# rvolden/C3POa

Measured on AMD Instinct MI355X. Metric: R2C2 reads->consensus/sec, higher is better.
Workload: dtype int32

## Files before the change

c3poa_amd/csrc/c3_args.h:

```cpp
#pragma once
#include "c3_dev.h"
#include <cstddef>

struct C3Counters {
  int queue;
  int peaks_queue;
  unsigned long long cells;
  unsigned long long cells_computed;
  unsigned long long zero_cells;
  int poa_ovf;
  int poa_ovf16;
  int n_windows;
  int win_ovf;
  int win_queue2;
  int band_layers, band_fallback;
  int band_mismatch;
  struct { int window, layer, R, q, band_row, full_row, next_row; } verify;
  unsigned long long phases[16];
};
static_assert(offsetof(C3Counters, cells) % 8 == 0 && offsetof(C3Counters, cells_computed) % 8 == 0 &&
              offsetof(C3Counters, zero_cells) % 8 == 0 && offsetof(C3Counters, phases) % 8 == 0, "u64 counters must be 8-byte aligned");

struct ConkArgs {
  C3Batch b; const uint8_t* sp_codes; const int* sp_len; int32_t* track; C3Info* info; C3Counters* cnt;
// ... 17 lines not shown
  int* overflow;
  int* overflow16;
};
#define C3_POA_NI 19
__host__ __device__ inline int c3_poa_far_shift(bool w32) { return w32 ? 0 : 2; }
struct PoaLayout { size_t ints, edges, cells, bases, score, desc, jump, path, total; };
__host__ __device__ inline PoaLayout c3_poa_layout(size_t Ncap, size_t K, int cells_cap, int far_shift, size_t Pcap) {
  PoaLayout l;
  l.ints = sizeof(int) * C3_POA_NI * Ncap; l.edges = sizeof(int) * 3 * Ncap * K;
  l.cells = 2 * (size_t)cells_cap + 16 * (size_t)(cells_cap >> far_shift);
  l.bases = 5 * Ncap; l.score = sizeof(long long) * Ncap; l.desc = sizeof(uint4) * 2 * Ncap;
  l.jump = sizeof(int) * C3_JUMP_LEVELS * Ncap; l.path = sizeof(int) * Pcap;
  l.total = l.ints + l.edges + l.cells + l.bases + l.score + l.desc + l.jump + l.path;
  return l;
}

struct WLayer { int qbeg, len, begin, end; };
struct WinRec { int rid, w, n_layers, blen, tgs, out_len, polished, pad_; };
struct PrepArgs {
  C3Batch b; C3Info* info; C3Params p; C3Counters* cnt; const int* work; int n_work;
  const uint8_t* draft; int32_t* tpos; int wcap; uint8_t* eD; int64_t ecap; int* lw_first; int* lw_last; int NLcap, NWcap;
  WinRec* wrec; WLayer* wlay; int* win_base;
  int sub_shift;
  int rows_old;
};
struct WinArgs {
  C3Batch b; C3Params p; C3Counters* cnt; int n_win; const WinRec* wrec_in; WinRec* wrec; const WLayer* wlay; int NLcap;
  const uint8_t* draft;
  uint8_t* base; int* ibase; int* ebase; long long* score;
  int32_t* H; uint16_t* D; uint4* rdesc; int Ncap, K; long long hcap; uint8_t* wout; int wout_cap;
  int Lcap;
  int band_mode;
  const int* wlist; int* ovf_list;
};
#define W_INTS 19
struct WinLayout { size_t ints, edges, bases, score, H, D, desc, total; };
__host__ __device__ inline WinLayout c3_win_layout(size_t Ncap, size_t K, size_t hcap) {
  WinLayout l;
  l.ints = sizeof(int) * W_INTS * Ncap; l.edges = sizeof(int) * 4 * Ncap * K; l.bases = 2 * Ncap; l.score = sizeof(long long) * Ncap;
  l.H = sizeof(int32_t) * hcap; l.D = hcap; l.desc = sizeof(uint4) * (Ncap + 1);
  l.total = l.ints + l.edges + l.bases + l.score + l.H + l.D + l.desc;
  return l;
}
struct StitchArgs {
  C3Batch b; C3Info* info; const int* work; int n_work; const WinRec* wrec; const int* win_base; const uint8_t* wout; int wout_cap; char* cons;
  const uint8_t* zflag;
};
struct AdapterArgs {
  C3Batch b; C3Params p; C3Counters* cnt;
  const uint8_t* ad_codes; const int* ad_len; int n_ad;
  uint8_t* D; long long dcap;
  int32_t* out;
};

struct ZeroArgs {
  C3Batch b; C3Info* info; C3Params p; C3Counters* cnt; const int* work; int n_work;
  uint8_t* D; long long dcap;
  int4* zinfo; uint8_t* zflag;
  const uint8_t* draft; char* cons;
  uint8_t* S; long long scap; int zk;
};

struct ZlLayout { long long ck, dir, car, total; };
__host__ __device__ inline ZlLayout c3_zl_layout(long long n0, long long n1, long long K) {
  ZlLayout l;
  l.ck = 0;
// ... 15 lines not shown
```

c3poa_amd/csrc/c3_stages.hip:

```cpp
#include "c3_host.h"

__global__ void k_summary(const C3Info* info, const int64_t* off, int n, Summary* out) {
  int i = blockIdx.x * blockDim.x + threadIdx.x;
  if (i >= n) return;
  const C3Info* p = &info[i];
  Summary s; s.status = p->status; s.n_sub = p->n_sub; s.max_sub = 0; s.sum_sub = 0; s.max_dang = 0; s.n_peaks = p->n_peaks;
  for (int k = 0; k < p->n_sub; ++k) { int l = p->sub_end[k] - p->sub_beg[k]; s.sum_sub += l; if (l > s.max_sub) s.max_sub = l; }
  int L = (int)(off[i + 1] - off[i]);
  s.front = p->has_front ? p->front_end : 0; s.tail = p->has_tail ? L - p->tail_beg : 0;
  if (p->has_front) s.max_dang = p->front_end;
  if (p->has_tail && L - p->tail_beg > s.max_dang) s.max_dang = L - p->tail_beg;
  out[i] = s;
}

static hipError_t zero_counters(c3_handle* h) { return hipMemsetAsync(h->d_counter.p, 0, sizeof(C3Counters), h->stream); }

static int auto_slots(c3_handle* h, int want, size_t per_slot_bytes, int n_items, int waves_per_cu) {
  int s = want > 0 ? want : h->n_cus * waves_per_cu;
  size_t budget = h->mem_total ? h->mem_total / 3 : ((size_t)64 << 30);
  if (per_slot_bytes > 0) { size_t mx = budget / per_slot_bytes; if ((size_t)s > mx) s = (int)std::max<size_t>(mx, 1); }
  if (s > n_items) s = std::max(n_items, 1);
  return s;
}

// ... 285 lines not shown
  h->n_windows = n_win;
  DBG("prep done: n_win=%d\n", n_win);
  const int wout_cap = 3 * WL + 64;
  HIPCHK(hipEventRecord(h->ev[7], h->stream));
  if (n_win > 0) {
    HIPCHK(h->d_wout.ensure((size_t)n_win * wout_cap));
    const int Ncap = 3 * WL + 40 * NLcap, K = NLcap + 2;
    const long long hcap_full = (long long)(Ncap + 1) * 64 * 12;
    const int R_typ = std::min(Ncap, WL + WL / 4 + 30 * NLcap + 64);
    long long hcap = std::min(hcap_full, (long long)(R_typ + R_typ / 2 + 4) * 256);
    if (const char* e = getenv("C3_DEBUG_HCAP_DIV")) hcap = std::max(4096LL, hcap_full / std::max(1, atoi(e)) / 64 * 64);
    const WinLayout L = c3_win_layout(Ncap, K, hcap), L2 = c3_win_layout(Ncap, K, hcap_full);
    const int slots = auto_slots(h, h->cfg.slots_win, L.total, n_win, 20);
    const int slots2 = hcap < hcap_full ? std::min(slots, 256) : 0;
    const size_t S = (size_t)slots, S2 = (size_t)slots2;
    HIPCHK(h->s_win_i.ensure(L.ints * S + 64)); HIPCHK(h->s_win_nk.ensure(L.edges * S));
    HIPCHK(h->s_win_h.ensure(L.H * S)); HIPCHK(h->s_win_d.ensure(L.D * S + 256));
    HIPCHK(h->s_win_b.ensure(L.bases * S)); HIPCHK(h->s_win_sc.ensure(L.score * S)); HIPCHK(h->s_win_desc.ensure(L.desc * S));
    if (slots2) {
      HIPCHK(h->s_win_h2.ensure(L2.H * S2)); HIPCHK(h->s_win_d2.ensure(L2.D * S2 + 256));
      HIPCHK(h->d_wovf.ensure(sizeof(int) * (size_t)n_win));
    }
    WinArgs a; memset(&a, 0, sizeof(a));
    a.b = dev_batch(h); a.p = dev_params(h->cfg); a.cnt = dev_cnt(h); a.n_win = n_win;
    a.wrec_in = h->d_wrec.as<WinRec>(); a.wrec = h->d_wrec.as<WinRec>(); a.wlay = h->d_wlay.as<WLayer>(); a.NLcap = NLcap;
    a.draft = h->d_draft.as<uint8_t>();
    a.ibase = h->s_win_i.as<int>(); a.ebase = h->s_win_nk.as<int>();
    a.base = h->s_win_b.as<uint8_t>(); a.score = h->s_win_sc.as<long long>();
    a.H = h->s_win_h.as<int32_t>(); a.D = h->s_win_d.as<uint16_t>(); a.rdesc = h->s_win_desc.as<uint4>(); a.Ncap = Ncap; a.K = K; a.hcap = hcap; a.Lcap = std::min(std::min(Ncap, 2 * WL + 30 * NLcap), ((getenv("C3_DEBUG_WIN_LDS") ? atoi(getenv("C3_DEBUG_WIN_LDS")) : 6656) - 16) / 6);
    if (const char* e = getenv("C3_DEBUG_WIN_LCAP")) a.Lcap = std::max(64, std::min(Ncap, atoi(e)));
    a.wout = h->d_wout.as<uint8_t>(); a.wout_cap = wout_cap;
    HIPCHK(zero_counters(h));
    if (const char* e = getenv("C3_DEBUG_BAND")) a.band_mode = !strcmp(e, "off") ? 1 : !strcmp(e, "fail") ? 2 : !strcmp(e, "verify") ? 3 : 0;
    a.ovf_list = slots2 ? h->d_wovf.as<int>() : nullptr;
    c3k_launch_window(&a, slots, h->stream);
    HIPCHK(hipGetLastError());
    if (slots2) {
      a.H = h->s_win_h2.as<int32_t>(); a.D = h->s_win_d2.as<uint16_t>(); a.hcap = hcap_full;
      a.wlist = h->d_wovf.as<int>(); a.ovf_list = nullptr;
      c3k_launch_window(&a, slots2, h->stream);
      HIPCHK(hipGetLastError());
    }
    HIPCHK(hipMemcpyAsync(h->phase_win, dev_cnt(h)->phases, sizeof(h->phase_win), hipMemcpyDeviceToHost, h->stream));
  }
  HIPCHK(hipEventRecord(h->ev[8], h->stream));
  StitchArgs s; memset(&s, 0, sizeof(s));
  s.b = dev_batch(h); s.info = h->d_info.as<C3Info>(); s.work = h->d_work.as<int>(); s.n_work = nw;
  s.wrec = h->d_wrec.as<WinRec>(); s.win_base = h->d_wbase.as<int>(); s.wout = h->d_wout.as<uint8_t>(); s.wout_cap = wout_cap;
  s.cons = h->d_cons.as<char>(); s.zflag = h->d_zflag.as<uint8_t>();
  DBG("stitch\n");
  c3k_launch_stitch(&s, std::min(nw, h->n_cus * 16), h->stream);
  HIPCHK(hipGetLastError());
  HIPCHK(hipEventRecord(h->ev[9], h->stream));
  HIPCHK(read_counters(h, &c));
  if (n_win > 0) {
    h->tm.n_win_redo = c.win_ovf; h->tm.cells_polish += c.cells; h->tm.cells_polish_computed += c.cells_computed;
    h->tm.n_band_layers = c.band_layers; h->tm.n_band_fallback = c.band_fallback; h->tm.n_band_mismatch = c.band_mismatch;
    if (c.band_mismatch) fprintf(stderr, "c3poa: band verify mismatch in window %d layer %d (R = %d): last differing base q = %d, band row %d, full row %d, row of q+1 = %d\n",
                                 c.verify.window, c.verify.layer, c.verify.R, c.verify.q, c.verify.band_row, c.verify.full_row, c.verify.next_row);
  }
  HIPCHK(hipEventElapsedTime(ms_prep, h->ev[5], h->ev[6]));
  HIPCHK(hipEventElapsedTime(ms_win, h->ev[7], h->ev[8]));
  HIPCHK(hipEventElapsedTime(ms_st, h->ev[8], h->ev[9]));
  h->tm.n_windows = n_win;
  return 0;
}
// ... 102 lines not shown
```

c3poa_amd/csrc/k_polish.hip:

```cpp
#include "c3_dev.h"
#include "c3_args.h"
#include "c3_launch.h"
#include <algorithm>
#include <type_traits>

#define WSYNC() __syncthreads()
#define EI(v, k) ((size_t)(k) * (size_t)c.Ncap + (size_t)(v))
#ifndef C3_WIN_RING
#define C3_WIN_RING 1
#endif



#ifndef C3_PREP_WAVES
#define C3_PREP_WAVES 5
#endif
#define EC 5
#define EXT_DCAP 4096
#define EXT_STATIC (-(1 << 27))
#define EXT_ECW 8
__device__ inline long long ext_dir_bytes(long long n, int rpw) { return (n / rpw + 1) * 256; }
template <bool DL>
__device__ long long extend_align(const PrepArgs& a, const uint32_t* pk, const uint8_t* draft, const uint8_t* ldraft, int C,
                                  int pb, int n, int dir_, int32_t* tpos, uint8_t* D, int lane) {
// ... 349 lines not shown
  __device__ __forceinline__ WArr<int> order2() const { return {I, (unsigned)(4 - osel) * (unsigned)Ncap}; }
  __device__ __forceinline__ WArr<int> lob() const { return {I, 17u * (unsigned)Ncap + 8u}; }
#undef W_I
  __device__ __forceinline__ WArr<int> in_from() const { return {E, 0u}; }
  __device__ __forceinline__ WArr<int> in_w() const { return {E, (unsigned)Ncap * (unsigned)K}; }
  __device__ __forceinline__ WArr<int> out_to() const { return {E, 2u * (unsigned)Ncap * (unsigned)K}; }
  __device__ __forceinline__ WArr<int> out_w() const { return {E, 3u * (unsigned)Ncap * (unsigned)K}; }
  __device__ __forceinline__ WArr<uint8_t> base() const { return {B8, 0u}; }
  __device__ __forceinline__ WArr<uint8_t> mask() const { return {B8, (unsigned)Ncap}; }
};

#ifndef WU
#define WU 4
#endif
__device__ void w_blocks(WCtx& c, int lane) {
  int gprev = -1;
  for (int i0 = 0; i0 < c.n; i0 += 64 * WU) {
    int v[WU], r[WU];
#pragma unroll
    for (int u = 0; u < WU; ++u) { const int i = i0 + 64 * u + lane; v[u] = i < c.n ? c.order()[i] : -1; }
#pragma unroll
    for (int u = 0; u < WU; ++u) r[u] = v[u] >= 0 ? c.grp()[v[u]] : -2;
#pragma unroll
    for (int u = 0; u < WU; ++u) {
      const int i = i0 + 64 * u + lane;
      const int rp = wave_shr1(r[u], gprev);
      gprev = wave_bcast(r[u], 63);
      if (v[u] >= 0 && r[u] != rp) { c.gfirst()[r[u]] = i; if (i > 0) c.glast()[rp] = i - 1; }
      if (v[u] >= 0 && i + 1 == c.n) c.glast()[r[u]] = i;
    }
  }
  WSYNC();
}
__device__ void w_reorder(WCtx& c, int n_old, int lane, int* lds, int lds_cap) {
  const int n_new = c.n - n_old;
  const bool inl = n_new <= lds_cap;
  if (inl) { for (int k = lane; k < n_new; k += 64) lds[k] = c.anchor()[k]; WSYNC(); }
  for (int i0 = 0; i0 < n_old; i0 += 64 * WU) {
    int v[WU];
#pragma unroll
    for (int u = 0; u < WU; ++u) { const int i = i0 + 64 * u + lane; v[u] = i < n_old ? c.order()[i] : -1; }
#pragma unroll
    for (int u = 0; u < WU; ++u) {
      const int i = i0 + 64 * u + lane;
      if (v[u] < 0) continue;
      int lo = 0, hi = n_new;
      if (inl) { while (lo < hi) { int m = (lo + hi) >> 1; if (lds[m] < i) lo = m + 1; else hi = m; } }
      else { while (lo < hi) { int m = (lo + hi) >> 1; if (c.anchor()[m] < i) lo = m + 1; else hi = m; } }
      c.order2()[i + lo] = v[u]; c.index()[v[u]] = i + lo;
    }
  }
  for (int k = lane; k < n_new; k += 64) { const int pos = (inl ? lds[k] : c.anchor()[k]) + 1 + k; c.order2()[pos] = n_old + k; c.index()[n_old + k] = pos; }
  c.osel ^= 1;
  WSYNC();
  w_blocks(c, lane);
}

__device__ void win_build_desc(WCtx& c, int R, int lane, unsigned long long* m2, unsigned long long* ma, bool allow2) {
  const int K = c.K;
  const WArr<int> kept = c.opn();
  int nkept = 0;
  for (int r0 = 1; r0 <= R; r0 += 64) {
    const int r = r0 + lane;
    bool two = false, adj = false;
    unsigned needh = 0;
    if (r <= R) {
      const int v = c.rows()[r];
      const int nin = c.n_in()[v];
      unsigned p[4] = {0, 0, 0, 0};
      int np = 0;
      for (int k = 0; k < nin; ++k) {
        const int pr = c.rowof()[c.in_from()[EI(v, k)]];
        if (pr < 0) continue;
        if (np < 4) p[np] = (unsigned)pr;
// ... 280 lines not shown
      const bool act = j <= Q;
      const int qc = (act && j >= 1) ? c3_code_at(pk, qbeg + j - 1) : 7;
      int bd = INT32_MIN, dd = 0, bv = INT32_MIN, dv = 0, np = 0;
      for (int k = 0; k <= nin; ++k) {
        int prow;
        if (k < nin) { prow = c.rowof()[c.in_from()[EI(v, k)]]; if (prow < 0) continue; ++np; }
        else { if (np > 0) break; prow = 0; }
        const int tt = min(np > 0 ? np - 1 : 0, 63);
        const int32_t* hp_ = c.H + (size_t)prow * RS;
        if (act) {
          if (j > 0) { int cnd = hp_[j - 1] + ((vb == qc) ? mt : mm); if (cnd > bd) { bd = cnd; dd = 255 - tt; } }
          int cv = hp_[j] + g;
          if (cv > bv) { bv = cv; dv = 191 - tt; }
        }
      }
      int hv = bd, dir = dd;
      if (bv > hv) { hv = bv; dir = dv; }
      const int y = act ? hv - g * j : C3_NEG2;
      const int s = wave_scan_max(y);
      const int ex = max(wave_shr1(s, C3_NEG2), carry);
      carry = max(carry, wave_bcast(s, 63));
      const int lf = ex + g * j;
      int hh = hv;
      if (j > 0 && lf > hh) { hh = lf; dir = W_TAG_H; }
      if (act) { hrow[j] = hh; drow[j] = (uint8_t)dir; }
      if (isend && j == Q) c.hend()[r] = hh;
    }
    WSYNC();
  }
  return 0;
}

#include "k_polish_band.h"
__host__ __device__ __forceinline__ int win_mask_words(int Ncap) { return ((Ncap + 64) >> 6) + 1; }
__host__ __device__ __forceinline__ size_t win_lds_bytes(int Lcap, int Ncap) {
  const size_t masks = (size_t)32 * win_mask_words(Ncap);
  const size_t a = (size_t)Lcap * 6 + 16, b = masks + 4 * 5 * 64 * 4 + 64, c = masks + 4 * (size_t)wb_lds_dwords(639, 4), d = masks + 4 * (size_t)(W_TBW + W_QCAP);
  size_t m = a > b ? a : b; m = m > c ? m : c; m = m > d ? m : d;
  return m;
}

__device__ __forceinline__ int win_idx(int j, int cpl) { return cpl ? (j / cpl) * ((cpl + 3) & ~3) + j % cpl : j; }

__device__ int win_rows_dispatch(WCtx& c, const C3Params& P, const uint32_t* pk, int qbeg, int Q, int R, int lane, int* cpl_out, int* rs_out, unsigned long long* dbg,
                                 unsigned long long* m2, unsigned long long* ma, unsigned long long* d0, unsigned long long* d1, int ring_off, int lds_ints, int begin, int end, int blen, int* cb_io, int* nblocks) {
  const int need = (Q + 1 + 63) / 64;
  int cpl;
  const int pm = max(max(abs(P.pol_match), abs(P.pol_mismatch)), abs(P.pol_gap));
  const bool ok16 = !(4 * pm * (max(R, Q) + 4) >= 31000 || 4 * (abs(P.pol_match) + abs(P.pol_gap)) * (Q + 4) >= 31000 || pm > 30 || P.pol_gap >= 0);
  if (!ok16) cpl = 0;
#ifdef C3_EXP_NOWIDE
  else if (need <= 2) cpl = 2; else if (need <= 4) cpl = 4; else cpl = 0;
#else
  else if (need <= 2) cpl = 2; else if (need <= 4) cpl = 4; else if (need <= 6) cpl = 6; else if (need <= 8) cpl = 8;
  else if (need <= 10) cpl = 10; else cpl = 0;
#endif
  const int span = end - begin + 1;
  int cb = R * 4 < span * 5 ? 2 : R * 2 < span * 3 ? 3 : 4;
  cb = max(cb, *cb_io);
  if (cb > 4) cb = 0;
  if (!*cb_io || !cb || !ok16 || need > 10 || need <= cb || span < 1 || max(P.pol_match, P.pol_mismatch) <= 0 || ring_off + wb_lds_dwords(Q, cb) > lds_ints) cb = 0;
#ifdef C3_BAND_OFF
  cb = 0;
#endif
#ifdef C3_PHASE_PROF
  const unsigned long long bd_t0 = __builtin_readcyclecounter();
#endif
  if (cb && !win_build_desc_band(c, R, Q, begin, end, blen, cb, lane, m2, ma, d0, d1, nblocks)) cb = 0;
#ifdef C3_EXP_X2_DESC
  if (cb && !win_build_desc_band(c, R, Q, begin, end, blen, cb, lane, m2, ma, d0, d1, nblocks)) cb = 0;
#endif
#ifdef C3_PHASE_PROF
  dbg[5] += __builtin_readcyclecounter() - bd_t0;
#endif
  *cb_io = cb;
  if (cb) {
    *cpl_out = cb; *rs_out = 256;
    int rc = 0;
#ifdef C3_EXP_X2_ROWS
    for (int rep_ = 0; rep_ < 2; ++rep_)
#endif
    switch (cb) {
      case 2: rc = win_rows_band<2>(c.I, c.E, c.H, c.D, c.rdesc, c.K, c.n, c.Ncap, c.hcap, P.pol_match, P.pol_mismatch, P.pol_gap, pk, qbeg, Q, R, dbg, ring_off, *nblocks); break;
      case 3: rc = win_rows_band<3>(c.I, c.E, c.H, c.D, c.rdesc, c.K, c.n, c.Ncap, c.hcap, P.pol_match, P.pol_mismatch, P.pol_gap, pk, qbeg, Q, R, dbg, ring_off, *nblocks); break;
      default: rc = win_rows_band<4>(c.I, c.E, c.H, c.D, c.rdesc, c.K, c.n, c.Ncap, c.hcap, P.pol_match, P.pol_mismatch, P.pol_gap, pk, qbeg, Q, R, dbg, ring_off, *nblocks); break;
    }
    if (rc < 0) return rc;
    if (rc > 0) c.lob()[0] = INT32_MAX;
    return 0;
  }
  *cpl_out = cpl; *rs_out = cpl ? 64 * ((cpl + 3) & ~3) : need * 64;
#ifdef C3_PHASE_PROF
  const unsigned long long bd_t1 = __builtin_readcyclecounter();
#endif
  win_build_desc(c, R, lane, m2, ma, cpl != 0);
#ifdef C3_PHASE_PROF
  dbg[5] += __builtin_readcyclecounter() - bd_t1;
#endif
  switch (cpl) {
    case 2: return win_rows<2>(c.I, c.E, c.H, c.D, c.rdesc, c.K, c.n, c.Ncap, c.hcap, P.pol_match, P.pol_mismatch, P.pol_gap, pk, qbeg, Q, R, dbg, ring_off);
    case 4: return win_rows<4>(c.I, c.E, c.H, c.D, c.rdesc, c.K, c.n, c.Ncap, c.hcap, P.pol_match, P.pol_mismatch, P.pol_gap, pk, qbeg, Q, R, dbg, ring_off);
#ifndef C3_EXP_NOWIDE
    case 6: return win_rows<6>(c.I, c.E, c.H, c.D, c.rdesc, c.K, c.n, c.Ncap, c.hcap, P.pol_match, P.pol_mismatch, P.pol_gap, pk, qbeg, Q, R, dbg, ring_off);
    case 8: return win_rows<8>(c.I, c.E, c.H, c.D, c.rdesc, c.K, c.n, c.Ncap, c.hcap, P.pol_match, P.pol_mismatch, P.pol_gap, pk, qbeg, Q, R, dbg, ring_off);
    case 10: return win_rows<10>(c.I, c.E, c.H, c.D, c.rdesc, c.K, c.n, c.Ncap, c.hcap, P.pol_match, P.pol_mismatch, P.pol_gap, pk, qbeg, Q, R, dbg, ring_off);
#endif
    default: return win_rows_lin(c, P, pk, qbeg, Q, R, lane);
  }
}

__device__ __forceinline__ int win_consensus(WCtx& c, int* s_score, unsigned short* s_pred, int tgs, int nl, uint8_t* out, int wout_cap, int lane) {
  int olen = 0;
  const int K = c.K, n = c.n;
  int max_id = 0, max_sc = -1;
  bool have_max = false;
  for (int c0 = 0; c0 < n; c0 += 64) {
    const int idx = c0 + lane;
    const bool live = idx < n;
    const int v = live ? c.order()[idx] : 0;
    const int nin = live ? c.n_in()[v] : 0;
    int bw = -1, bu = -1, cm = 0;
    {
      const int w0 = c.in_w()[EI(v, 0)], w1 = c.in_w()[EI(v, 1)], u0 = c.in_from()[EI(v, 0)], u1 = c.in_from()[EI(v, 1)];
      if (nin > 0) { bw = w0; bu = u0; cm = 1; }
      if (nin > 1) { if (w1 > bw) { bw = w1; bu = u1; cm = 1; } else if (w1 == bw) ++cm; }
    }
    for (int k = 2; __builtin_amdgcn_ballot_w64(k < nin) != 0; ++k) {
      if (k < nin) {
// ... 115 lines not shown
    int wi = 0;
    if (lane == 0) {
      if (SECOND) {
        wi = atomicAdd(&a.cnt->win_queue2, 1);
        wi = wi < *(const volatile int*)&a.cnt->win_ovf ? a.wlist[wi] : -1;
      } else {
        wi = atomicAdd(&a.cnt->queue, 1);
        if (wi >= a.n_win) wi = -1;
      }
    }
    wi = wave_first(wi);
    if (wi < 0) break;
    PH_MARK(9)
    const WinRec rec = a.wrec_in[wi];
    const int rid = rec.rid, blen = rec.blen, nl = rec.n_layers;
    const int64_t off = a.b.off[rid];
    const uint32_t* pk = a.b.pk + a.b.woff[rid];
    const uint8_t* qual = a.b.qual + off;
    const uint8_t* bb = a.draft + off + (size_t)rec.w * P.pol_window;
    uint8_t* out = a.wout + (size_t)wi * a.wout_cap;
    const WLayer* lay = a.wlay + (size_t)wi * a.NLcap;
    long long cells = 0, cells_done = 0;
    int olen = 0, polished = 0, fail = 0, n_band = 0, n_fallback = 0;
    if (nl + 1 < 3) {
      if (blen > a.wout_cap) fail = 1;
      else { for (int i = lane; i < blen; i += 64) out[i] = bb[i]; olen = blen; }
    } else {
      c.osel = 0;
      for (int i = lane; i < blen; i += 64) {
        c.base()[i] = bb[i]; c.grp()[i] = i; c.order()[i] = i; c.index()[i] = i; c.ncov()[i] = 1;
        c.n_in()[i] = i > 0; c.n_out()[i] = i + 1 < blen;
        if (i > 0) { c.in_from()[EI(i, 0)] = i - 1; c.in_w()[EI(i, 0)] = 0; }
        if (i + 1 < blen) { c.out_to()[EI(i, 0)] = i + 1; c.out_w()[EI(i, 0)] = 0; }
      }
      c.n = blen;
      WSYNC();
      w_blocks(c, lane);
      PH_MARK(0)
      const int offset = (int)(0.01 * (double)blen);
      const int lbeg = lane < nl ? lay[min(lane, nl - 1)].begin : INT32_MAX;
      int lrank = 0;
      if (nl <= 64) for (int y = 0; y < nl; ++y) { const int by = __builtin_amdgcn_readlane(lbeg, y); lrank += (by < lbeg) || (by == lbeg && y < lane); }
      for (int t = 0; t < nl && !fail; ++t) {
        int li = -1;
        if (nl <= 64) li = __builtin_ctzll(__ballot(lane < nl && lrank == t) | (1ull << 63));
        else for (int x = 0; x < nl; ++x) {
          int before = 0;
          for (int y = 0; y < nl; ++y) before += (lay[y].begin < lay[x].begin) || (lay[y].begin == lay[x].begin && y < x);
          if (before == t) { li = x; break; }
        }
        const WLayer l = lay[li];
        const int Q = l.len;
        const bool full = l.begin < offset && l.end > blen - offset;
        if (!full) {
          const int K = c.K;
          const int eidx = c.glast()[c.grp()[l.end]];
          const WArr<int> gseed = c.rowof();
          for (int i = lane; i < c.n; i += 64) { const int v = c.order()[i]; c.mask()[v] = (v >= l.begin && i <= eidx) ? 1 : 0; }
          WSYNC();
          for (;;) {
            for (int v0 = 0; v0 < c.n; v0 += 64 * WU) {
              int m_[WU], g_[WU];
#pragma unroll
              for (int u = 0; u < WU; ++u) { const int v = min(v0 + 64 * u + lane, c.n - 1); m_[u] = c.mask()[v]; g_[u] = c.grp()[v]; }
#pragma unroll
              for (int u = 0; u < WU; ++u) if (v0 + 64 * u + lane < c.n && m_[u]) gseed[g_[u]] = 0;
            }
            WSYNC();
            for (int v0 = 0; v0 < c.n; v0 += 64 * WU) {
              int m_[WU], g_[WU], no_[WU], t0_[WU], t1_[WU], s0_[WU], s1_[WU];
#pragma unroll
              for (int u = 0; u < WU; ++u) {
                const int v = min(v0 + 64 * u + lane, c.n - 1);
                m_[u] = c.mask()[v]; g_[u] = c.grp()[v]; no_[u] = c.n_out()[v]; t0_[u] = c.out_to()[EI(v, 0)]; t1_[u] = c.out_to()[EI(v, 1)];
              }
#pragma unroll
              for (int u = 0; u < WU; ++u) {
                s0_[u] = c.mask()[min(max(t0_[u], 0), c.Ncap - 1)]; s1_[u] = c.mask()[min(max(t1_[u], 0), c.Ncap - 1)];
              }
#pragma unroll
              for (int u = 0; u < WU; ++u) {
                const int v = v0 + 64 * u + lane;
                if (v >= c.n || !m_[u]) continue;
                int seed = v == l.end || (no_[u] > 0 && s0_[u]) || (no_[u] > 1 && s1_[u]);
                for (int k = 2; k < no_[u] && !seed; ++k) seed = c.mask()[c.out_to()[EI(v, k)]];
                if (seed) gseed[g_[u]] = 1;
              }
            }
            WSYNC();
            int changed = 0;
            for (int v0 = 0; v0 < c.n; v0 += 64 * WU) {
              int m_[WU], g_[WU], gs_[WU];
#pragma unroll
              for (int u = 0; u < WU; ++u) { const int v = min(v0 + 64 * u + lane, c.n - 1); m_[u] = c.mask()[v]; g_[u] = c.grp()[v]; }
#pragma unroll
              for (int u = 0; u < WU; ++u) gs_[u] = gseed[g_[u]];
#pragma unroll
              for (int u = 0; u < WU; ++u) { const int v = v0 + 64 * u + lane; if (v < c.n && m_[u] && !gs_[u]) { c.mask()[v] = 0; changed = 1; } }
            }
            changed = __ballot(changed) != 0;
            WSYNC();
            if (!changed) break;
          }
        }
        PH_MARK(1)
        int R = 0;
#ifdef C3_EXP_X2_COMP
        for (int rep_ = 0; rep_ < 2; ++rep_) { R = 0;
#endif
        for (int i0 = 0; i0 < c.n; i0 += 64 * WU) {
          int v[WU]; bool in[WU];
#pragma unroll
          for (int u = 0; u < WU; ++u) { const int i = i0 + 64 * u + lane; v[u] = i < c.n ? c.order()[i] : -1; }
#pragma unroll
          for (int u = 0; u < WU; ++u) in[u] = v[u] >= 0 && (full || c.mask()[v[u]]);
#pragma unroll
          for (int u = 0; u < WU; ++u) {
            const unsigned long long bal = __ballot(in[u]);
            if (v[u] >= 0) {
              if (in[u]) { int r = R + 1 + __popcll(bal & ((1ull << lane) - 1)); c.rows()[r] = v[u]; c.rowof()[v[u]] = r; }
              else c.rowof()[v[u]] = -1;
            }
            R += __popcll(bal);
          }
        }
#ifdef C3_EXP_X2_COMP
        WSYNC(); }
#endif
        WSYNC();
        PH_MARK(2)
        const int ring_off = 8 * MW;
        const QArr rq = {(unsigned short*)((unsigned*)lds_dyn + ring_off + W_TBW), c.opq(), Q > W_QCAP};
        const QArr tq = {(unsigned short*)((unsigned*)lds_dyn + ring_off + W_TBW) + W_QCAP, c.opn(), Q > W_QCAP};
        unsigned long long tbp_[4] = {0, 0, 0, 0};
        bool verify = false;
        for (int vpass = 0; vpass < 2 && !fail; ++vpass) {
        int cpl = 0, RS = 0, cb = a.band_mode != 1 && vpass == 0, gbs = INT32_MIN, gbr = 0;
        for (int attempt = 0; attempt < 4; ++attempt) {
          unsigned long long dbg_[6] = {0, 0, 0, 0, 0, 0};
          int nblocks = 0;
          if (win_rows_dispatch(c, P, pk, l.qbeg, Q, R, lane, &cpl, &RS, dbg_, m2bits, mabits, d0bits, d1bits, ring_off, lds_ints, l.begin, l.end, blen, &cb, &nblocks) < 0) { fail = SECOND ? 1 : 2; break; }
#ifdef C3_PHASE_PROF
          ph_acc_[10] += dbg_[0]; ph_acc_[11] += dbg_[1];
#endif
          PH_MARK(3)
          cells_done += (long long)(R + 1) * (cb ? 64 * cb : Q + 1);
          if (cb) {
            WSYNC();
            const int bound = c.lob()[0];
            gbs = c.lob()[1]; gbr = c.lob()[2];
#ifdef C3_EXP_NOCERT
            if (cb) { ++n_band; break; }
#endif
            if (gbs != INT32_MIN && bound < gbs && a.band_mode != 2) { ++n_band; break; }
          } else {
            int bs = INT32_MIN, br = INT32_MAX / 2;
            for (int r = 1 + lane; r <= R; r += 64) { const int sc = c.hend()[r]; if (sc > bs) { bs = sc; br = r; } }
            gbs = wave_max(bs);
            gbr = wave_min(bs == gbs ? br : INT32_MAX / 2);
            break;
          }
          ++n_fallback; cb = (cb < 4 && a.band_mode == 0) ? cb + 1 : 0;
        }
        if (fail) break;
        cells += (long long)(R + 1) * (Q + 1);
        PH_MARK(4)
#ifdef C3_PHASE_PROF
        unsigned long long tbc_[3] = {0, 0, 0};
#endif
#ifdef C3_EXP_X2_TB
        for (int tbrep = 0; tbrep < 2; ++tbrep)
#endif
        if (cb) win_traceback_band(c.I, c.E, c.D, c.rdesc, c.K, c.n, c.Ncap, cb, R, Q, (gbs == INT32_MIN) ? 0 : gbr, MW, Q > W_QCAP, tbp_);
        else
// ... 69 lines not shown
              }
              if (r <= 0 || j <= 0) break;
              const int drift = (jt - j) - (rt - r);
              if (rt - r >= 64 || drift > 5 || drift < -5) break;
            }
            WSYNC();
          }
        }
        if (!(a.band_mode == 3 && vpass == 0 && cb)) break;
        verify = true;
        WSYNC();
        for (int q = lane; q < Q; q += 64) c.opq()[q] = rq.get(q);
        WSYNC();
        }
        if (verify && !fail) {
          int diff = 0;
          for (int q = lane; q < Q; q += 64) diff |= c.opq()[q] != rq.get(q);
          const unsigned long long dm = __ballot(diff);
          if (dm != 0) {
            int qd = -1;
            for (int q = lane; q < Q; q += 64) if (c.opq()[q] != rq.get(q)) qd = q;
            qd = wave_max(qd);
            if (lane == 0) { atomicAdd(&a.cnt->band_mismatch, 1); a.cnt->verify.window = wi; a.cnt->verify.layer = t; a.cnt->verify.R = R; a.cnt->verify.q = qd;
                             a.cnt->verify.band_row = c.opq()[qd]; a.cnt->verify.full_row = rq.get(qd); a.cnt->verify.next_row = qd + 1 < Q ? rq.get(qd + 1) : -1; }
          }
        }
        WSYNC();
        if (fail) break;
        PH_MARK(5)
#ifdef C3_PHASE_PROF
        ph_acc_[12] += tbp_[0]; ph_acc_[13] += tbp_[1]; ph_acc_[14] += tbp_[2]; ph_acc_[15] += tbp_[3];
#endif
        const int n_old = c.n;
        int carry_anchor = -1, carry_new = 0;
        for (int q0 = 0; q0 < Q; q0 += 128) {
          int v_[2], cb_[2], rr_[2], bs_[2], anc_[2], gf_[2], tgt_[2], gnew_[2];
          bool act_[2];
#pragma unroll
          for (int h2 = 0; h2 < 2; ++h2) {
            const int q = q0 + 64 * h2 + lane;
            act_[h2] = q < Q;
            const int r = act_[h2] ? rq.get(q) : 0;
            v_[h2] = r > 0 ? c.rows()[r] : -1;
            cb_[h2] = act_[h2] ? c3_code_at(pk, l.qbeg + q) : 0;
          }
#pragma unroll
          for (int h2 = 0; h2 < 2; ++h2) { const int vv = max(v_[h2], 0); rr_[h2] = c.grp()[vv]; bs_[h2] = c.base()[vv]; }
#pragma unroll
          for (int h2 = 0; h2 < 2; ++h2) { anc_[h2] = c.glast()[rr_[h2]]; gf_[h2] = c.gfirst()[rr_[h2]]; }
#pragma unroll
          for (int h2 = 0; h2 < 2; ++h2) {
            int tgt = -1, gnew = -1;
            if (v_[h2] >= 0) {
              if (bs_[h2] == cb_[h2]) tgt = v_[h2];
              else for (int i = gf_[h2]; i <= anc_[h2]; ++i) { int x = c.order()[i]; if (c.base()[x] == cb_[h2]) { tgt = x; break; } }
              if (tgt < 0) gnew = rr_[h2];
            } else anc_[h2] = -1;
            tgt_[h2] = tgt; gnew_[h2] = gnew;
          }
#pragma unroll
          for (int h2 = 0; h2 < 2; ++h2) {
            const int q = q0 + 64 * h2 + lane;
            if (q0 + 64 * h2 >= Q) break;
            const bool act = act_[h2];
            const int cb = cb_[h2], gnew = gnew_[h2], anc = anc_[h2];
            int tgt = tgt_[h2];
            const int isnew = act && tgt < 0;
            const int as = max(wave_scan_max(anc), carry_anchor);
            carry_anchor = wave_bcast(as, 63);
            const int ps = wave_scan_add(isnew);
            const int k = carry_new + ps - isnew;
            carry_new += wave_bcast(ps, 63);
            if (isnew) {
              const int id = n_old + k;
              if (id < c.Ncap) {
                c.base()[id] = (uint8_t)cb; c.n_in()[id] = 0; c.n_out()[id] = 0; c.grp()[id] = gnew >= 0 ? gnew : id; c.ncov()[id] = 0;
                c.anchor()[k] = as;
              }
              tgt = id;
            }
            if (act) tq.set(q, tgt);
          }
        }
        const int nn = n_old + carry_new;
        if (nn > c.Ncap) { fail = 1; break; }
        WSYNC();
        const int K = c.K;
        for (int q0 = 0; q0 < Q; q0 += 128) {
          int v_[2], u_[2], w_[2], no_[2], ni_[2], nc_[2], o0_[2], o1_[2], i0_[2], i1_[2];
          bool ed_[2];
#pragma unroll
          for (int h2 = 0; h2 < 2; ++h2) {
            const int q = q0 + 64 * h2 + lane;
            const bool act = q < Q;
            ed_[h2] = act && q > 0;
            v_[h2] = act ? tq.get(q) : 0;
            u_[h2] = ed_[h2] ? tq.get(q - 1) : 0;
            const int qq = l.qbeg + (ed_[h2] ? q : 1);
            w_[h2] = ((int)qual[qq - 1] - 33) + ((int)qual[qq] - 33);
          }
#pragma unroll
          for (int h2 = 0; h2 < 2; ++h2) {
            nc_[h2] = c.ncov()[v_[h2]]; no_[h2] = c.n_out()[u_[h2]]; ni_[h2] = c.n_in()[v_[h2]];
            o0_[h2] = c.out_to()[EI(u_[h2], 0)]; o1_[h2] = c.out_to()[EI(u_[h2], 1)];
            i0_[h2] = c.in_from()[EI(v_[h2], 0)]; i1_[h2] = c.in_from()[EI(v_[h2], 1)];
          }
#pragma unroll
          for (int h2 = 0; h2 < 2; ++h2) {
            const int q = q0 + 64 * h2 + lane;
            if (q < Q) c.ncov()[v_[h2]] = nc_[h2] + 1;
            if (!ed_[h2]) continue;
            const int u = u_[h2], v = v_[h2], w = w_[h2], no = no_[h2], ni = ni_[h2];
            int hit = (no > 0 && o0_[h2] == v) ? 0 : (no > 1 && o1_[h2] == v) ? 1 : -1;
            if (hit < 0) for (int k = 2; k < no; ++k) if (c.out_to()[EI(u, k)] == v) { hit = k; break; }
            if (hit >= 0) {
              int hin = (ni > 0 && i0_[h2] == u) ? 0 : (ni > 1 && i1_[h2] == u) ? 1 : -1;
              if (hin < 0) for (int t2 = 2; t2 < ni; ++t2) if (c.in_from()[EI(v, t2)] == u) { hin = t2; break; }
              c.out_w()[EI(u, hit)] += w;
              if (hin >= 0) c.in_w()[EI(v, hin)] += w;
            } else {
              c.out_to()[EI(u, no)] = v; c.out_w()[EI(u, no)] = w; c.n_out()[u] = no + 1;
              c.in_from()[EI(v, ni)] = u; c.in_w()[EI(v, ni)] = w; c.n_in()[v] = ni + 1;
            }
          }
        }
        WSYNC();
        c.n = nn;
        PH_MARK(6)
        w_reorder(c, n_old, lane, lds_dyn, lds_ints);
        PH_MARK(7)
      }
      if (!fail) {
        if (c.n <= a.Lcap) olen = win_consensus(c, s_score, s_pred, rec.tgs, nl, out, a.wout_cap, lane);
        else olen = win_consensus(c, (int*)c.H, (unsigned short*)(c.H + c.Ncap), rec.tgs, nl, out, a.wout_cap, lane);
        PH_MARK(8)
        if (olen < 0) { fail = 1; olen = 0; } else polished = 1;
      }
    }
    if (fail == 2 && a.ovf_list) {
      if (lane == 0) a.ovf_list[atomicAdd(&a.cnt->win_ovf, 1)] = wi;
    } else if (lane == 0) {
      WinRec* r = &a.wrec[wi];
      r->out_len = fail ? -1 : olen; r->polished = polished;
      atomicAdd(&a.cnt->cells, (unsigned long long)cells);
      atomicAdd(&a.cnt->cells_computed, (unsigned long long)cells_done);
      if (n_band) atomicAdd(&a.cnt->band_layers, n_band);
      if (n_fallback) atomicAdd(&a.cnt->band_fallback, n_fallback);
    }
    WSYNC();
  }
  PH_FLUSH(a.cnt->phases)
}


__global__ __launch_bounds__(64) void k_stitch(StitchArgs a) {
  const int lane = wave_lane();
  for (int wi = blockIdx.x; wi < a.n_work; wi += gridDim.x) {
    const int rid = a.work[wi];
    C3Info* info = &a.info[rid];
    if (info->status != C3_ST_OK) continue;
    if (a.zflag && a.zflag[rid]) continue;
    const int64_t off = a.b.off[rid];
// ... 28 lines not shown
```

c3poa_amd/csrc/k_polish_band.h:

```cpp
#pragma once

#define WB_PADL 4
#define WB_PADR 28
#define WB_MAXSHIFT 24
#ifndef WB_RING
#define WB_RING 4
#endif
#define WB_EROW 12
#define WB_EROWS 32
__host__ __device__ __forceinline__ int wb_slot_shorts(int cb) { return WB_PADL + 64 * cb + WB_PADR; }
__host__ __device__ __forceinline__ int wb_lds_dwords(int Q, int cb) { return ((Q + 2) & ~1) + WB_RING * wb_slot_shorts(cb) / 2 + WB_EROWS * WB_EROW / 2; }
__device__ __forceinline__ int wb_left(int cb) { return cb == 2 ? 70 : cb == 3 ? 105 : 140; }
__host__ __device__ __forceinline__ int wb_rpw(int cb) { return cb == 2 ? 8 : 4; }
__host__ __device__ __forceinline__ int wb_bit0(int cb) { return 32 - 2 * cb * wb_rpw(cb); }

__device__ __forceinline__ int wb_words(int R, int cb) { return (R + wb_rpw(cb) - 1) / wb_rpw(cb); }

#define WB_W_LO(w) ((int)((w) & 0x3ffu))
#define WB_W_DIST(w) ((int)(((w) >> 10) & 0xffu))
#define WB_W_BIDX(w) ((int)((w) >> 18))
__device__ int win_build_desc_band(WCtx& c, int R, int Q, int begin, int end, int blen, int CB, int lane,
                                   unsigned long long* m2, unsigned long long* ma, unsigned long long* d0, unsigned long long* d1, int* nblocks) {
  const int BW = 64 * CB, WLf = wb_left(CB), span = end - begin + 1, lomax = Q + 1 - BW;
  if (R >= 16000 || Q > 1000) return 0;
// ... 64 lines not shown
#pragma unroll
        for (int k = 0; k < 4; ++k) if (pe[u][k] >= 0) { p[np < 4 ? np : 3] = (unsigned)pe[u][k]; ++np; }
        for (int k = 4; k < nin[u]; ++k) { const int pr = c.rowof()[c.in_from()[EI(v[u], k)]]; if (pr >= 0) { if (np < 4) p[np] = (unsigned)pr; ++np; } }
#pragma unroll
        for (int k = 0; k < 4; ++k) if (se[u][k] >= 0) { has = 1; dist = max(dist, se[u][k] - r); if (se[u][k] == r + 1) next = 1; else other = 1; }
        for (int k = 4; k < nout[u]; ++k) {
          const int sr = c.rowof()[c.out_to()[EI(v[u], k)]];
          if (sr >= 0) { has = 1; dist = max(dist, sr - r); if (sr == r + 1) next = 1; else other = 1; }
        }
        far = dist > WB_RING;
        if (dist > 64) bad = 1;
        ovf = np > 4; virt = np == 0;
        if (np == 0) np = 1;
        two = np == 1;
        adj = two && (int)p[0] == r - 1;
        fast = adj && !far && has && dl <= 1;
#ifdef C3_EXP_NOFAST
        fast = 0;
#endif
      }
      const unsigned fastn = (unsigned)__builtin_amdgcn_update_dpp(0, (int)fast, 0x130, 0xf, 0xf, false);
      if (live) {
        const unsigned wr = other | (next & (fastn ^ 1u));
        uint4 d; d.x = vb[u] * 8u | ((unsigned)min(np, 255) << 8) | (ovf << 16) | (far << 17) | ((has ^ 1u) << 18) | ((unsigned)two << 19) | (fast << 20)
                       | ((unsigned)(fast ? dl : 0) << 22) | (wr << 23) | (virt << 24);
        d.y = p[0] | (p[1] << 16); d.z = p[2] | (p[3] << 16); d.w = (unsigned)lo | ((unsigned)min(dist, 255) << 10) | ((unsigned)bidx << 18);
        c.rdesc[r] = d;
      }
      const unsigned long long b2 = __ballot(two), ba = __ballot(adj), bd0 = __ballot(dl & 1), bd1 = __ballot((dl & 2) != 0);
      if (lane == 0) { m2[r0 >> 6] = b2; ma[r0 >> 6] = ba; d0[r0 >> 6] = bd0; d1[r0 >> 6] = bd1; }
    }
  }
  *nblocks = nbc;
  bad = __ballot(bad) != 0;
  WSYNC();
  return !bad;
}

template <int CB>
__device__ __forceinline__ void wb_park_edge(unsigned eaddr, const int (&h)[CB]) {
  const unsigned long long emask = 0x8000000000000003ull;
  if (CB == 2)
    asm volatile("s_mov_b64 exec, %0\n\tds_write_b16 %1, %2\n\tds_write_b16 %1, %3 offset:2\n\ts_mov_b64 exec, -1"
                 :: "s"(emask), "v"(eaddr), "v"(h[0]), "v"(h[CB > 1 ? 1 : 0]) : "memory");
  else if (CB == 3)
    asm volatile("s_mov_b64 exec, %0\n\tds_write_b16 %1, %2\n\tds_write_b16 %1, %3 offset:2\n\tds_write_b16 %1, %4 offset:4\n\ts_mov_b64 exec, -1"
                 :: "s"(emask), "v"(eaddr), "v"(h[0]), "v"(h[CB > 1 ? 1 : 0]), "v"(h[CB > 2 ? 2 : 0]) : "memory");
  else
    asm volatile("s_mov_b64 exec, %0\n\tds_write_b16 %1, %2\n\tds_write_b16 %1, %3 offset:2\n\tds_write_b16 %1, %4 offset:4\n\tds_write_b16 %1, %5 offset:6\n\ts_mov_b64 exec, -1"
                 :: "s"(emask), "v"(eaddr), "v"(h[0]), "v"(h[CB > 1 ? 1 : 0]), "v"(h[CB > 2 ? 2 : 0]), "v"(h[CB > 3 ? 3 : 0]) : "memory");
}

template <int CB>
__device__ __attribute__((noinline)) int win_rows_band(int* cI, int* cE, int32_t* cH, uint8_t* cD, uint4* crdesc, int cK, int cn, int cNcap, long long chcap,
                                                       int mt_, int mm_, int g_, const uint32_t* pk_, int qbeg_, int Q_, int R_, unsigned long long* dbg_, int lds_off_, int nblocks_) {
  WCtx c;
  c.I = uni_ptr(cI); c.E = uni_ptr(cE); c.B8 = nullptr; c.score = nullptr; c.H = uni_ptr(cH); c.D = uni_ptr(cD);
  c.rdesc = uni_ptr(crdesc); c.K = uni32(cK); c.n = uni32(cn); c.Ncap = uni32(cNcap);
  c.hcap = ((long long)uni32((int)(chcap >> 32)) << 32) | (unsigned)uni32((int)chcap);
  const uint32_t* pk = uni_ptr(pk_);
  unsigned long long* dbg = uni_ptr(dbg_);
  const int qbeg = uni32(qbeg_), Q = uni32(Q_), R = uni32(R_), NB = uni32(nblocks_);
  const int lane = wave_lane();
  extern __shared__ int lds_dyn[];
  constexpr int BW = 64 * CB, SLOT = WB_PADL + BW + WB_PADR , HS = BW + 8 ;
  constexpr int RPW = CB == 2 ? 8 : 4, BPR = 2 * CB, BIT0 = 32 - BPR * RPW;
// ... 381 lines not shown
```

Measured before the change: 424,000.

## Add chain fast path for first window layer over linear backbone graph

For the first layer of each polishing window, when the graph is still the linear draft backbone, the kernel now builds row descriptors directly from the chain (including a banded variant), skips topological/group bookkeeping, and uses a specialized fuse routine that appends new nodes and edges without group lookups. It also skips w_blocks at window init and uses identity order in reorder for chain layers. This is meant to remove generic graph traversal, row collection and descriptor-building costs for the common first alignment. In exchange it adds code paths that must stay consistent with the general graph invariants, and it can be disabled through an environment variable.

```diff
diff --git a/c3poa_amd/csrc/c3_args.h b/c3poa_amd/csrc/c3_args.h
--- a/c3poa_amd/csrc/c3_args.h
+++ b/c3poa_amd/csrc/c3_args.h
@@ -73,6 +73,7 @@
   int Lcap;
   int band_mode;
   const int* wlist; int* ovf_list;
+  int no_chain;
 };
 #define W_INTS 19
 struct WinLayout { size_t ints, edges, bases, score, H, D, desc, total; };
diff --git a/c3poa_amd/csrc/c3_stages.hip b/c3poa_amd/csrc/c3_stages.hip
--- a/c3poa_amd/csrc/c3_stages.hip
+++ b/c3poa_amd/csrc/c3_stages.hip
@@ -341,6 +341,7 @@
     a.wout = h->d_wout.as<uint8_t>(); a.wout_cap = wout_cap;
     HIPCHK(zero_counters(h));
     if (const char* e = getenv("C3_DEBUG_BAND")) a.band_mode = !strcmp(e, "off") ? 1 : !strcmp(e, "fail") ? 2 : !strcmp(e, "verify") ? 3 : 0;
+    if (const char* e = getenv("C3_DEBUG_WIN_CHAIN")) a.no_chain = !strcmp(e, "0");
     a.ovf_list = slots2 ? h->d_wovf.as<int>() : nullptr;
     c3k_launch_window(&a, slots, h->stream);
     HIPCHK(hipGetLastError());
diff --git a/c3poa_amd/csrc/k_polish.hip b/c3poa_amd/csrc/k_polish.hip
--- a/c3poa_amd/csrc/k_polish.hip
+++ b/c3poa_amd/csrc/k_polish.hip
@@ -405,14 +405,14 @@
   }
   WSYNC();
 }
-__device__ void w_reorder(WCtx& c, int n_old, int lane, int* lds, int lds_cap) {
+__device__ void w_reorder(WCtx& c, int n_old, int lane, int* lds, int lds_cap, bool ident) {
   const int n_new = c.n - n_old;
   const bool inl = n_new <= lds_cap;
   if (inl) { for (int k = lane; k < n_new; k += 64) lds[k] = c.anchor()[k]; WSYNC(); }
   for (int i0 = 0; i0 < n_old; i0 += 64 * WU) {
     int v[WU];
 #pragma unroll
-    for (int u = 0; u < WU; ++u) { const int i = i0 + 64 * u + lane; v[u] = i < n_old ? c.order()[i] : -1; }
+    for (int u = 0; u < WU; ++u) { const int i = i0 + 64 * u + lane; v[u] = i < n_old ? (ident ? i : c.order()[i]) : -1; }
 #pragma unroll
     for (int u = 0; u < WU; ++u) {
       const int i = i0 + 64 * u + lane;
@@ -759,6 +759,112 @@
 }
 
 #include "k_polish_band.h"
+
+
+__device__ __attribute__((noinline)) void win_chain_desc(int* cI, uint4* crdesc, int cNcap, const uint8_t* bb_, int v0_, int R_, int allow2_, int mw_) {
+  WCtx c;
+  c.I = uni_ptr(cI); c.Ncap = uni32(cNcap);
+  uint4* const rdesc = uni_ptr(crdesc);
+  const uint8_t* const bb = uni_ptr(bb_);
+  const int v0 = uni32(v0_), R = uni32(R_), MW = uni32(mw_);
+  const unsigned two = uni32(allow2_) != 0;
+  const int lane = wave_lane();
+  extern __shared__ int lds_dyn[];
+  unsigned long long* m2 = (unsigned long long*)lds_dyn; unsigned long long* ma = m2 + MW;
+  for (int r0 = 1; r0 <= R; r0 += 64) {
+    const int r = r0 + lane;
+    if (r <= R) {
+      typedef unsigned u32x4 __attribute__((ext_vector_type(4)));
+      u32x4 d;
+      d.x = (unsigned)GP(const uint8_t, bb)[v0 + r - 1] | (1u << 8) | ((unsigned)(r == R) << 18) | (two << 19) | ((two & (unsigned)(r < R)) << 20);
+      d.y = (unsigned)(r - 1); d.z = 0; d.w = 0;
+      GP(u32x4, rdesc)[r] = d;
+      GP(int, c.hend().ptr())[r] = INT32_MIN;
+      GP(int, c.opn().ptr())[r] = 0;
+    }
+    const unsigned long long bl = two ? __ballot(r <= R) : 0ull;
+    if (lane == 0) { m2[r0 >> 6] = bl; ma[r0 >> 6] = bl; }
+  }
+  WSYNC();
+}
+
+__device__ __attribute__((noinline)) int win_chain_fuse(int* cI, int* cE, uint8_t* cB8, int cK, int cNcap, const uint8_t* bb_, const uint32_t* pk_, const uint8_t* qual_,
+                                                        int qbeg_, int Q_, int v0_, int blen_, int ring_off_) {
+  WCtx c;
+  c.I = uni_ptr(cI); c.E = uni_ptr(cE); c.B8 = uni_ptr(cB8); c.K = uni32(cK); c.Ncap = uni32(cNcap);
+  const uint8_t* const bb = uni_ptr(bb_);
+  const uint32_t* const pk = uni_ptr(pk_);
+  const uint8_t* const qual = uni_ptr(qual_);
+  const int qbeg = uni32(qbeg_), Q = uni32(Q_), v0 = uni32(v0_), blen = uni32(blen_), ring_off = uni32(ring_off_);
+  const int lane = wave_lane();
+  extern __shared__ int lds_dyn[];
+  const QArr rq = {(unsigned short*)((unsigned*)lds_dyn + ring_off + W_TBW), c.opq(), Q > W_QCAP};
+  const QArr tq = {(unsigned short*)((unsigned*)lds_dyn + ring_off + W_TBW) + W_QCAP, c.opn(), Q > W_QCAP};
+  int* const gI = c.I; int* const gE = c.E;
+  const unsigned N = (unsigned)c.Ncap, NK = N * (unsigned)c.K;
+#define CI_(k, i) GP(int, gI)[(unsigned)(k) * N + (unsigned)(i)]
+#define CE_(a, v, k) GP(int, gE)[(unsigned)(a) * NK + (unsigned)(k) * N + (unsigned)(v)]
+  int carry_anchor = -1, carry_new = 0;
+  for (int q0 = 0; q0 < Q; q0 += 128) {
+    int v_[2], cb_[2], bs_[2];
+    bool act_[2];
+#pragma unroll
+    for (int h2 = 0; h2 < 2; ++h2) {
+      const int q = q0 + 64 * h2 + lane;
+      act_[h2] = q < Q;
+      const int r = act_[h2] ? rq.get(q) : 0;
+      v_[h2] = r > 0 ? v0 + r - 1 : -1;
+      cb_[h2] = act_[h2] ? c3_code_at(pk, qbeg + q) : 0;
+      bs_[h2] = (int)GP(const uint8_t, bb)[max(v_[h2], 0)];
+    }
+#pragma unroll
+    for (int h2 = 0; h2 < 2; ++h2) {
+      const int q = q0 + 64 * h2 + lane;
+      if (q0 + 64 * h2 >= Q) break;
+      const bool act = act_[h2];
+      const int v = v_[h2], cb = cb_[h2];
+      int tgt = (v >= 0 && bs_[h2] == cb) ? v : -1;
+      const int isnew = act && tgt < 0;
+      const int as = max(wave_scan_max(v), carry_anchor);
+      carry_anchor = wave_bcast(as, 63);
+      const int ps = wave_scan_add(isnew);
+      const int k = carry_new + ps - isnew;
+      carry_new += wave_bcast(ps, 63);
+      if (isnew) {
+        const int id = blen + k;
+        if (id < c.Ncap) {
+          GP(uint8_t, c.B8)[id] = (uint8_t)cb; CI_(0, id) = 0; CI_(1, id) = 0; CI_(2, id) = v >= 0 ? v : id; CI_(8, id) = 0;
+          CI_(10, k) = as;
+        }
+        tgt = id;
+      }
+      if (act) tq.set(q, tgt);
+    }
+  }
+  const int nn = blen + carry_new;
+  if (nn > c.Ncap) return nn;
+  WSYNC();
+  for (int q0 = 0; q0 < Q; q0 += 64) {
+    const int q = q0 + lane;
+    const bool act = q < Q, ed = act && q > 0;
+    const int v = act ? tq.get(q) : 0, u = ed ? tq.get(q - 1) : 0;
+    const int qq = qbeg + (ed ? q : 1);
+    const int w = ((int)GP(const uint8_t, qual)[qq - 1] - 33) + ((int)GP(const uint8_t, qual)[qq] - 33);
+    if (act) CI_(8, v) = (v < blen) + 1;
+    if (!ed) continue;
+    if (v < blen && v == u + 1) { CE_(3, u, 0) = w; CE_(1, v, 0) = w; }
+    else {
+      const int no = u + 1 < blen, ni = v < blen && v > 0;
+      CE_(2, u, no) = v; CE_(3, u, no) = w; CI_(1, u) = no + 1;
+      CE_(0, v, ni) = u; CE_(1, v, ni) = w; CI_(0, v) = ni + 1;
+    }
+  }
+#undef CI_
+#undef CE_
+  WSYNC();
+  return nn;
+}
+
 __host__ __device__ __forceinline__ int win_mask_words(int Ncap) { return ((Ncap + 64) >> 6) + 1; }
 __host__ __device__ __forceinline__ size_t win_lds_bytes(int Lcap, int Ncap) {
   const size_t masks = (size_t)32 * win_mask_words(Ncap);
@@ -770,7 +876,7 @@
 __device__ __forceinline__ int win_idx(int j, int cpl) { return cpl ? (j / cpl) * ((cpl + 3) & ~3) + j % cpl : j; }
 
 __device__ int win_rows_dispatch(WCtx& c, const C3Params& P, const uint32_t* pk, int qbeg, int Q, int R, int lane, int* cpl_out, int* rs_out, unsigned long long* dbg,
-                                 unsigned long long* m2, unsigned long long* ma, unsigned long long* d0, unsigned long long* d1, int ring_off, int lds_ints, int begin, int end, int blen, int* cb_io, int* nblocks) {
+                                 unsigned long long* m2, unsigned long long* ma, unsigned long long* d0, unsigned long long* d1, int ring_off, int lds_ints, int begin, int end, int blen, int* cb_io, int* nblocks, const uint8_t* chain_bb, int chain_v0, int MW) {
   const int need = (Q + 1 + 63) / 64;
   int cpl;
   const int pm = max(max(abs(P.pol_match), abs(P.pol_mismatch)), abs(P.pol_gap));
@@ -793,7 +899,8 @@
 #ifdef C3_PHASE_PROF
   const unsigned long long bd_t0 = __builtin_readcyclecounter();
 #endif
-  if (cb && !win_build_desc_band(c, R, Q, begin, end, blen, cb, lane, m2, ma, d0, d1, nblocks)) cb = 0;
+  if (cb && chain_bb) { *nblocks = R; if (!win_chain_desc_band(c.rdesc, chain_bb, chain_v0, R, Q, begin, end, cb, MW)) cb = 0; }
+  else if (cb && !win_build_desc_band(c, R, Q, begin, end, blen, cb, lane, m2, ma, d0, d1, nblocks)) cb = 0;
 #ifdef C3_EXP_X2_DESC
   if (cb && !win_build_desc_band(c, R, Q, begin, end, blen, cb, lane, m2, ma, d0, d1, nblocks)) cb = 0;
 #endif
@@ -820,7 +927,15 @@
 #ifdef C3_PHASE_PROF
   const unsigned long long bd_t1 = __builtin_readcyclecounter();
 #endif
-  win_build_desc(c, R, lane, m2, ma, cpl != 0);
+  if (chain_bb && cpl) win_chain_desc(c.I, c.rdesc, c.Ncap, chain_bb, chain_v0, R, 1, MW);
+  else {
+    if (chain_bb) {
+      for (int v = lane; v < c.n; v += 64) c.rowof()[v] = (v >= chain_v0 && v < chain_v0 + R) ? v - chain_v0 + 1 : -1;
+      for (int r = 1 + lane; r <= R; r += 64) c.rows()[r] = chain_v0 + r - 1;
+      WSYNC();
+    }
+    win_build_desc(c, R, lane, m2, ma, cpl != 0);
+  }
 #ifdef C3_PHASE_PROF
   dbg[5] += __builtin_readcyclecounter() - bd_t1;
 #endif
@@ -1002,10 +1117,11 @@
         c.n_in()[i] = i > 0; c.n_out()[i] = i + 1 < blen;
         if (i > 0) { c.in_from()[EI(i, 0)] = i - 1; c.in_w()[EI(i, 0)] = 0; }
         if (i + 1 < blen) { c.out_to()[EI(i, 0)] = i + 1; c.out_w()[EI(i, 0)] = 0; }
+        if (!a.no_chain) { c.gfirst()[i] = i; c.glast()[i] = i; }
       }
       c.n = blen;
       WSYNC();
-      w_blocks(c, lane);
+      if (a.no_chain) w_blocks(c, lane);
       PH_MARK(0)
       const int offset = (int)(0.01 * (double)blen);
       const int lbeg = lane < nl ? lay[min(lane, nl - 1)].begin : INT32_MAX;
@@ -1022,7 +1138,9 @@
         const WLayer l = lay[li];
         const int Q = l.len;
         const bool full = l.begin < offset && l.end > blen - offset;
-        if (!full) {
+        const bool chain = t == 0 && !a.no_chain && c.n == blen && l.begin >= 0 && l.begin <= l.end && l.end < blen;
+        const int chain_v0 = full ? 0 : l.begin;
+        if (!full && !chain) {
           const int K = c.K;
           const int eidx = c.glast()[c.grp()[l.end]];
           const WArr<int> gseed = c.rowof();
@@ -1074,11 +1192,11 @@
           }
         }
         PH_MARK(1)
-        int R = 0;
+        int R = chain ? (full ? blen : l.end - l.begin + 1) : 0;
 #ifdef C3_EXP_X2_COMP
-        for (int rep_ = 0; rep_ < 2; ++rep_) { R = 0;
-#endif
-        for (int i0 = 0; i0 < c.n; i0 += 64 * WU) {
+        for (int rep_ = 0; rep_ < 2; ++rep_) { if (!chain) R = 0;
+#endif
+        for (int i0 = 0; i0 < c.n && !chain; i0 += 64 * WU) {
           int v[WU]; bool in[WU];
 #pragma unroll
           for (int u = 0; u < WU; ++u) { const int i = i0 + 64 * u + lane; v[u] = i < c.n ? c.order()[i] : -1; }
@@ -1109,7 +1227,7 @@
         for (int attempt = 0; attempt < 4; ++attempt) {
           unsigned long long dbg_[6] = {0, 0, 0, 0, 0, 0};
           int nblocks = 0;
-          if (win_rows_dispatch(c, P, pk, l.qbeg, Q, R, lane, &cpl, &RS, dbg_, m2bits, mabits, d0bits, d1bits, ring_off, lds_ints, l.begin, l.end, blen, &cb, &nblocks) < 0) { fail = SECOND ? 1 : 2; break; }
+          if (win_rows_dispatch(c, P, pk, l.qbeg, Q, R, lane, &cpl, &RS, dbg_, m2bits, mabits, d0bits, d1bits, ring_off, lds_ints, l.begin, l.end, blen, &cb, &nblocks, chain ? bb : nullptr, chain_v0, MW) < 0) { fail = SECOND ? 1 : 2; break; }
 #ifdef C3_PHASE_PROF
           ph_acc_[10] += dbg_[0]; ph_acc_[11] += dbg_[1];
 #endif
@@ -1245,6 +1363,11 @@
         ph_acc_[12] += tbp_[0]; ph_acc_[13] += tbp_[1]; ph_acc_[14] += tbp_[2]; ph_acc_[15] += tbp_[3];
 #endif
         const int n_old = c.n;
+        int nn;
+        if (chain) {
+          nn = win_chain_fuse(c.I, c.E, c.B8, c.K, c.Ncap, bb, pk, qual, l.qbeg, Q, chain_v0, blen, ring_off);
+          if (nn > c.Ncap) { fail = 1; break; }
+        } else {
         int carry_anchor = -1, carry_new = 0;
         for (int q0 = 0; q0 < Q; q0 += 128) {
           int v_[2], cb_[2], rr_[2], bs_[2], anc_[2], gf_[2], tgt_[2], gnew_[2];
@@ -1295,7 +1418,7 @@
             if (act) tq.set(q, tgt);
           }
         }
-        const int nn = n_old + carry_new;
+        nn = n_old + carry_new;
         if (nn > c.Ncap) { fail = 1; break; }
         WSYNC();
         const int K = c.K;
@@ -1338,9 +1461,10 @@
           }
         }
         WSYNC();
+        }
         c.n = nn;
         PH_MARK(6)
-        w_reorder(c, n_old, lane, lds_dyn, lds_ints);
+        w_reorder(c, n_old, lane, lds_dyn, lds_ints, chain);
         PH_MARK(7)
       }
       if (!fail) {
diff --git a/c3poa_amd/csrc/k_polish_band.h b/c3poa_amd/csrc/k_polish_band.h
--- a/c3poa_amd/csrc/k_polish_band.h
+++ b/c3poa_amd/csrc/k_polish_band.h
@@ -120,6 +120,47 @@
     }
   }
   *nblocks = nbc;
+  bad = __ballot(bad) != 0;
+  WSYNC();
+  return !bad;
+}
+
+__device__ __attribute__((noinline)) int win_chain_desc_band(uint4* crdesc, const uint8_t* bb_, int v0_, int R_, int Q_, int begin_, int end_, int CB_, int mw_) {
+  uint4* const rdesc = uni_ptr(crdesc);
+  const uint8_t* const bb = uni_ptr(bb_);
+  const int v0 = uni32(v0_), R = uni32(R_), Q = uni32(Q_), begin = uni32(begin_), end = uni32(end_), CB = uni32(CB_), MW = uni32(mw_);
+  const int lane = wave_lane();
+  extern __shared__ int lds_dyn[];
+  unsigned long long* m2 = (unsigned long long*)lds_dyn; unsigned long long* ma = m2 + MW;
+  unsigned long long* d0 = ma + MW; unsigned long long* d1 = d0 + MW;
+  const int BW = 64 * CB, WLf = wb_left(CB), span = end - begin + 1, lomax = Q + 1 - BW;
+  if (R >= 16000 || Q > 1000) return 0;
+  int loc = 0, bad = 0;
+  for (int rb = 1; rb <= R; rb += 64) {
+    const int r = rb + lane;
+    const bool live = r <= R;
+    const unsigned vb = live ? (unsigned)GP(const uint8_t, bb)[v0 + r - 1] & 3u : 0u;
+    const int bbs = max(v0 + min(r, R) - 1, begin - 1);
+    const int cen = (int)(((long long)(bbs - begin + 1) * Q + span / 2) / span);
+    const int lo = min(max(cen - WLf, 0), lomax);
+    const int lop = wave_shr1(lo, loc);
+    loc = wave_bcast(lo, 63);
+    const int dl = live ? lo - lop : 0;
+    if (dl > 3) bad = 1;
+    const unsigned has = live && r < R;
+    const unsigned fast = has && dl <= 1;
+    const unsigned fastn = (unsigned)__builtin_amdgcn_update_dpp(0, (int)fast, 0x130, 0xf, 0xf, false);
+    if (live) {
+      const unsigned wr = has & (fastn ^ 1u);
+      typedef unsigned u32x4 __attribute__((ext_vector_type(4)));
+      u32x4 d;
+      d.x = vb * 8u | (1u << 8) | ((has ^ 1u) << 18) | (1u << 19) | (fast << 20) | ((fast ? (unsigned)dl : 0u) << 22) | (wr << 23) | ((unsigned)(r == 1) << 24);
+      d.y = (unsigned)(r - 1); d.z = 0; d.w = (unsigned)lo | (has << 10) | ((unsigned)r << 18);
+      GP(u32x4, rdesc)[r] = d;
+    }
+    const unsigned long long bl = __ballot(live), bd0 = __ballot(dl & 1), bd1 = __ballot((dl & 2) != 0);
+    if (lane == 0) { m2[rb >> 6] = bl; ma[rb >> 6] = bl; d0[rb >> 6] = bd0; d1[rb >> 6] = bd1; }
+  }
   bad = __ballot(bad) != 0;
   WSYNC();
   return !bad;
```

New measurement: 428,300 (median of 6 runs). 1.01x the previous value.
